# selftok-team/SelftokTokenizer

Hardware: NVIDIA H100
Metric: images/sec encode+50-step decode, 256x256/512-tok (higher is better)
Workload: dtype fp16 (IEEE-half operands on wgmma, fp32 accumulate; encoder/VQ/tables fp32)

## Files before the change

selftoktokenizer_b200/csrc/gemm_tc.cu:

```cuda
#include "common.cuh"
#include "hopper.cuh"
#include "kernels.h"

#include <stdlib.h>

namespace stk {

namespace {

using namespace hop;

constexpr int BM = 128, BN = 256, BK = 64, WK = 16;
constexpr int A_TILE_BYTES = BM * BK * 2;
constexpr int B_TILE_BYTES = BN * BK * 2;
constexpr int CONSUMERS = 2;
constexpr int NUM_THREADS = CONSUMERS * 128 + 128;
constexpr int PRODUCER_REGS = 40, CONSUMER_REGS = 232;
constexpr int ACC = BN / 2;
constexpr int kPrefetchKBlocks = 4;

template <int NSPLIT> struct Cfg {
  static constexpr int PLANES = NSPLIT == 3 ? 2 : 1;
  static constexpr int STAGE_BYTES = PLANES * (A_TILE_BYTES + B_TILE_BYTES);
  static constexpr int STAGES = NSPLIT == 3 ? 2 : 4;
  static constexpr int SMEM_BYTES = STAGES * STAGE_BYTES + 1024  + 256 ;
};

__device__ __forceinline__ void wgmma_tile(float (&d)[ACC], uint64_t da, uint64_t db, uint32_t acc, bool fp16) {
  if (fp16) wgmma_m64n256k16_ss_f16(d, da, db, acc);
  else wgmma_m64n256k16_ss_bf16(d, da, db, acc);
}

__device__ __forceinline__ float2 ldg2(const float* p) { return *reinterpret_cast<const float2*>(p); }

struct EpiRows {
  int orow[2], mrow[2];
  bool valid[2];
};

__device__ __forceinline__ EpiRows epilogue_rows(const Epilogue& e, int64_t row0, int64_t M) {
  const bool per_row_gate = e.mode == EPI_RESID && e.gate && (e.gate_period > 1 || e.tab_rows);
  const bool per_row_add = e.mode == EPI_STORE && e.addtab;
  EpiRows rw;
#pragma unroll
  for (int r = 0; r < 2; ++r) {
    const int64_t m = row0 + 8 * r;
    rw.valid[r] = m < M;
    const int mi = (int)m;
    rw.orow[r] = 0;
    if (e.row_map && rw.valid[r]) {
      rw.orow[r] = e.row_map[mi];
    } else if (e.plan && rw.valid[r]) {
      const int b = mi / e.rpb_in;
      const int n_img = e.rpb_out - (e.plan_ctx ? e.rpb_in : e.row_off);
      rw.orow[r] = b * e.rpb_out + plan_slot_row(mi % e.rpb_in, e.plan[2 * b], e.plan[2 * b + 1], n_img, e.plan_ctx != 0);
    } else if (rw.valid[r]) {
      rw.orow[r] = e.rpb_in > 0 ? (mi / e.rpb_in) * e.rpb_out + e.row_off + (mi % e.rpb_in) : mi;
    }
    if (e.tab_rows && rw.valid[r]) rw.mrow[r] = e.tab_rows[mi];
    else rw.mrow[r] = per_row_gate ? mi % e.gate_period : (per_row_add ? mi % e.add_period : 0);
  }
  return rw;
}

__device__ __forceinline__ void epilogue_prefetch(const Epilogue& e, const EpiRows& rw, int col0, int N) {
  if (e.mode != EPI_RESID) return;
  const int c0 = col0 & ~(BN - 1);
  const int q = (col0 >> 1) & 3;
#pragma unroll
  for (int r = 0; r < 2; ++r) {
#pragma unroll
    for (int h = 0; h < 2; ++h) {
      const int n = c0 + 32 * (2 * q + h);
      if (rw.valid[r] && n < N) prefetch_l2(e.resid + (int64_t)rw.orow[r] * e.ldo + n);
    }
  }
}

template <int MODE, bool GELU>
__device__ __forceinline__ void epilogue_tile(const Epilogue& e, const float (&acc)[ACC], const EpiRows& rw, int col0, int N) {
  constexpr int CH = MODE == EPI_RESID ? 4 : 8;
  const bool per_row_gate = MODE == EPI_RESID && e.gate && (e.gate_period > 1 || e.tab_rows);
  const bool per_row_add = MODE == EPI_STORE && e.addtab;
  const bool fp16 = e.fp16 != 0;
  const float2 zero = make_float2(0.f, 0.f), one = make_float2(1.f, 1.f);
#pragma unroll
  for (int c = 0; c < BN / 8; c += CH) {
    float2 bias[CH], res[2][CH], gt[2][CH], add[2][CH];
#pragma unroll
    for (int i = 0; i < CH; ++i) {
      const int n = col0 + 8 * (c + i);
      const bool in = n < N;
      bias[i] = e.bias && in ? ldg2(e.bias + n) : zero;
#pragma unroll
      for (int r = 0; r < 2; ++r) {
        const bool v = in && rw.valid[r];
        const int64_t o = (int64_t)rw.orow[r] * e.ldo + n;
        if (MODE == EPI_RESID) {
          res[r][i] = v ? ldg2(e.resid + o) : zero;
          gt[r][i] = v && e.gate ? ldg2(per_row_gate ? e.gate + (int64_t)rw.mrow[r] * e.gate_ld + n : e.gate + n) : one;
        }
        if (MODE == EPI_STORE) add[r][i] = v && per_row_add ? ldg2(e.addtab + (int64_t)rw.mrow[r] * e.add_ld + n) : zero;
      }
    }
#pragma unroll
    for (int i = 0; i < CH; ++i) {
      const int j = c + i;
      const int n = col0 + 8 * j;
      if (n >= N) continue;
#pragma unroll
      for (int r = 0; r < 2; ++r) {
        if (!rw.valid[r]) continue;
        float2 y = make_float2(acc[4 * j + 2 * r] + bias[i].x, acc[4 * j + 2 * r + 1] + bias[i].y);
        if (GELU) y = gelu_tanh_fast2(y);
        const int64_t o = (int64_t)rw.orow[r] * e.ldo + n;
        if (MODE == EPI_RESID) {
          y.x = fmaf(gt[r][i].x, y.x, res[r][i].x); y.y = fmaf(gt[r][i].y, y.y, res[r][i].y);
        }
        if (MODE == EPI_SPLIT) {
          const uint32_t hi = pack2_sat16(y.x, y.y, fp16);
          *reinterpret_cast<uint32_t*>(e.out_hi + o) = hi;
          if (e.out_lo) {
            const float lx = y.x - __bfloat162float(__float2bfloat16_rn(y.x)), ly = y.y - __bfloat162float(__float2bfloat16_rn(y.y));
            *reinterpret_cast<uint32_t*>(e.out_lo + o) = pack2_sat16(lx, ly, false);
          }
        } else {
          if (per_row_add) { y.x += add[r][i].x; y.y += add[r][i].y; }
          *reinterpret_cast<float2*>(e.out + o) = y;
        }
      }
    }
  }
}

__device__ __forceinline__ void epilogue_dispatch(const Epilogue& e, const float (&acc)[ACC], const EpiRows& rw, int col0, int N) {
  if (e.mode == EPI_RESID) epilogue_tile<EPI_RESID, false>(e, acc, rw, col0, N);
  else if (e.mode == EPI_SPLIT) {
    if (e.act == ACT_GELU) epilogue_tile<EPI_SPLIT, true>(e, acc, rw, col0, N);
    else epilogue_tile<EPI_SPLIT, false>(e, acc, rw, col0, N);
  } else {
    if (e.act == ACT_GELU) epilogue_tile<EPI_STORE, true>(e, acc, rw, col0, N);
    else epilogue_tile<EPI_STORE, false>(e, acc, rw, col0, N);
  }
}

struct TcMaps {
  CUtensorMap a_hi, a_lo, b_hi, b_lo;
};

struct GemmParams {
  int64_t M;
  int N, K;
  int fp16;
  Epilogue ep;
  int conv_C = 0, conv_H = 0, conv_W = 0, conv_stride = 1;
  int raster_gm = 4;
};

__device__ __forceinline__ void tile_coords(int t, int pm_tiles, int n_tiles, int GM, int& pm, int& n_blk) {
  const int per_group = GM * n_tiles;
  const int group = t / per_group;
  const int first = group * GM;
  const int gm = min(GM, pm_tiles - first);
  const int local = t - group * per_group;
  pm = first + local % gm;
  n_blk = local / gm;
}

template <int NSPLIT, int CL, bool FP16>
__global__ void __launch_bounds__(NUM_THREADS, 1)
gemm_tc_kernel(const __grid_constant__ TcMaps maps0, const __grid_constant__ TcMaps maps1, const GemmParams p0, const GemmParams p1) {
  static_assert(NSPLIT == 1 || !FP16, "the fp16 mode is single-pass");
  using C = Cfg<NSPLIT>;
  extern __shared__ uint8_t smem_raw[];
  const uint32_t smem_base = (smem_u32(smem_raw) + 1023u) & ~1023u;
  const uint32_t bar_base = smem_base + C::STAGES * C::STAGE_BYTES;
  auto full_bar = [&](int s) { return bar_base + 8u * s; };
  auto empty_bar = [&](int s) { return bar_base + 8u * (C::STAGES + s); };

  const int warp = threadIdx.x >> 5, lane = threadIdx.x & 31;
  const uint32_t rank = CL > 1 ? cluster_ctarank() : 0;
  const int pm_tiles0 = (int)((p0.M + CL * BM - 1) / (CL * BM)), n_tiles0 = (p0.N + BN - 1) / BN;
  const int pm_tiles1 = (int)((p1.M + CL * BM - 1) / (CL * BM)), n_tiles1 = (p1.N + BN - 1) / BN;
  const int tiles0 = pm_tiles0 * n_tiles0;
  const int num_tiles = tiles0 + pm_tiles1 * n_tiles1;
  const int cluster_id = blockIdx.x / CL, num_clusters = gridDim.x / CL;

  if (warp == CONSUMERS * 4 && lane == 0) {
    tma_prefetch_desc(&maps0.a_hi);
    tma_prefetch_desc(&maps0.b_hi);
    if (NSPLIT == 3) { tma_prefetch_desc(&maps0.a_lo); tma_prefetch_desc(&maps0.b_lo); }
    if (p1.M > 0) {
      tma_prefetch_desc(&maps1.a_hi);
      tma_prefetch_desc(&maps1.b_hi);
      if (NSPLIT == 3) { tma_prefetch_desc(&maps1.a_lo); tma_prefetch_desc(&maps1.b_lo); }
    }
    for (int s = 0; s < C::STAGES; ++s) { mbar_init(full_bar(s), 1); mbar_init(empty_bar(s), CONSUMERS * CL); }
    asm volatile("fence.mbarrier_init.release.cluster;" ::: "memory");
  }
  __syncthreads();
  if (CL > 1) cluster_sync_all();

  if (warp >= CONSUMERS * 4) {
    setmaxnreg_dec<PRODUCER_REGS>();
    if (warp == CONSUMERS * 4 && lane == 0) {
      int stage = 0; uint32_t phase = 0;
      const uint64_t w_policy = l2_policy_evict_last();
      for (int t = cluster_id; t < num_tiles; t += num_clusters) {
        const bool second = t >= tiles0;
        const TcMaps& mp = second ? maps1 : maps0;
        const GemmParams& pp = second ? p1 : p0;
        int pm, n_blk;
        if (second) tile_coords(t - tiles0, pm_tiles1, n_tiles1, p1.raster_gm, pm, n_blk);
        else tile_coords(t, pm_tiles0, n_tiles0, p0.raster_gm, pm, n_blk);
        const int nk = (pp.K + BK - 1) / BK;
        const int m_row = (pm * CL + (int)rank) * BM;
        const int n_row = n_blk * BN + (int)rank * (BN / CL);
        const int chunks = pp.conv_C > 0 ? pp.conv_C / BK : 1;
        int cx = 0, cy = 0, cb = 0;
        if (pp.conv_C > 0) {
          cx = m_row % pp.conv_W;
          cy = (m_row / pp.conv_W) % pp.conv_H;
          cb = m_row / (pp.conv_W * pp.conv_H);
        }
        for (int kb = 0; kb < nk; ++kb) {
          mbar_wait(empty_bar(stage), phase ^ 1);
          const uint32_t sa = smem_base + stage * C::STAGE_BYTES;
          const uint32_t sb = sa + C::PLANES * A_TILE_BYTES + (uint32_t)rank * (B_TILE_BYTES / CL);
          const uint32_t fb = full_bar(stage);
          mbar_expect_tx(fb, C::STAGE_BYTES);
          if (pp.conv_C > 0) {
            const int tap = kb / chunks, c0 = (kb - tap * chunks) * BK;
            const int dy = tap / 3, dx = tap - dy * 3;
            int x0 = cx + dx - 1, y0 = cy + dy - 1, n0 = cb;
            if (pp.conv_stride == 2) { x0 = cx + (dx >> 1); y0 = cy + (dy >> 1); n0 = cb * 4 + (dy & 1) * 2 + (dx & 1); }
            tma_load_4d(sa, &mp.a_hi, fb, c0, x0, y0, n0);
            if (NSPLIT == 3) tma_load_4d(sa + A_TILE_BYTES, &mp.a_lo, fb, c0, x0, y0, n0);
          } else {
            tma_load_2d(sa, &mp.a_hi, fb, kb * BK, m_row);
            if (NSPLIT == 3) tma_load_2d(sa + A_TILE_BYTES, &mp.a_lo, fb, kb * BK, m_row);
          }
          if (CL > 1) {
            tma_load_2d_mc(sb, &mp.b_hi, fb, kb * BK, n_row, (uint16_t)((1u << CL) - 1), w_policy);
            if (NSPLIT == 3) tma_load_2d_mc(sb + B_TILE_BYTES, &mp.b_lo, fb, kb * BK, n_row, (uint16_t)((1u << CL) - 1), w_policy);
          } else {
            tma_load_2d_hint(sb, &mp.b_hi, fb, kb * BK, n_row, w_policy);
            if (NSPLIT == 3) tma_load_2d_hint(sb + B_TILE_BYTES, &mp.b_lo, fb, kb * BK, n_row, w_policy);
          }
          if (++stage == C::STAGES) { stage = 0; phase ^= 1; }
        }
      }
    }
  } else {
    setmaxnreg_inc<CONSUMER_REGS>();
    const int wg = warp >> 2;
    const bool signaller = (threadIdx.x & 127) == 0;
    auto release = [&](int s) {
      if (!signaller) return;
      if (CL == 1) mbar_arrive(empty_bar(s));
      else for (int r = 0; r < CL; ++r) mbar_arrive_cluster(empty_bar(s), (uint32_t)r);
    };
    int stage = 0; uint32_t phase = 0;
    for (int t = cluster_id; t < num_tiles; t += num_clusters) {
      const bool second = t >= tiles0;
      int pm, n_blk;
      if (second) tile_coords(t - tiles0, pm_tiles1, n_tiles1, p1.raster_gm, pm, n_blk);
      else tile_coords(t, pm_tiles0, n_tiles0, p0.raster_gm, pm, n_blk);
      const int nk = ((second ? p1.K : p0.K) + BK - 1) / BK;
      const int wl = threadIdx.x & 127;
      const int64_t row0 = (int64_t)(pm * CL + (int)rank) * BM + wg * 64 + (wl >> 5) * 16 + ((wl & 31) >> 2);
      const int col0 = n_blk * BN + 2 * (wl & 3);
      const EpiRows rw = second ? epilogue_rows(p1.ep, row0, p1.M) : epilogue_rows(p0.ep, row0, p0.M);
      const int pf_kb = nk > kPrefetchKBlocks ? nk - kPrefetchKBlocks : 0;
      float acc[ACC];
#pragma unroll
      for (int i = 0; i < ACC; ++i) acc[i] = 0.f;
      int prev = -1;
      for (int kb = 0; kb < nk; ++kb) {
        mbar_wait(full_bar(stage), phase);
        const uint32_t sa_hi = smem_base + stage * C::STAGE_BYTES + wg * (64 * 128);
        const uint32_t sa_lo = sa_hi + A_TILE_BYTES;
        const uint32_t sb_hi = smem_base + stage * C::STAGE_BYTES + C::PLANES * A_TILE_BYTES;
        const uint32_t sb_lo = sb_hi + B_TILE_BYTES;
        wgmma_fence();
#pragma unroll
        for (int k = 0; k < BK / WK; ++k) {
          const uint32_t koff = k * WK * 2;
          const uint64_t da_hi = make_smem_desc(sa_hi + koff), db_hi = make_smem_desc(sb_hi + koff);
          wgmma_tile(acc, da_hi, db_hi, (kb > 0 || k > 0) ? 1u : 0u, FP16);
          if (NSPLIT == 3) {
            const uint64_t da_lo = make_smem_desc(sa_lo + koff), db_lo = make_smem_desc(sb_lo + koff);
            wgmma_tile(acc, da_hi, db_lo, 1u, false);
            wgmma_tile(acc, da_lo, db_hi, 1u, false);
          }
        }
        wgmma_commit();
        if (kb == pf_kb) {
          if (!second) epilogue_prefetch(p0.ep, rw, col0, p0.N);
          else epilogue_prefetch(p1.ep, rw, col0, p1.N);
        }
        wgmma_wait<1>();
        if (prev >= 0) release(prev);
        prev = stage;
        if (++stage == C::STAGES) { stage = 0; phase ^= 1; }
      }
      wgmma_wait<0>();
      fence_regs(acc);
      release(prev);
      if (!second) epilogue_dispatch(p0.ep, acc, rw, col0, p0.N);
      else epilogue_dispatch(p1.ep, acc, rw, col0, p1.N);
    }
  }
  if (CL > 1) cluster_sync_all();
}

typedef CUresult (*EncodeTiledFn)(CUtensorMap*, CUtensorMapDataType, cuuint32_t, void*, const cuuint64_t*, const cuuint64_t*,
                                  const cuuint32_t*, const cuuint32_t*, CUtensorMapInterleave, CUtensorMapSwizzle,
                                  CUtensorMapL2promotion, CUtensorMapFloatOOBfill);
EncodeTiledFn g_encode = nullptr;
constexpr int kMaxDev = 64;
int g_num_sms_dev[kMaxDev];
bool g_attr_dev[kMaxDev];
int g_raster_gm = 4;
int g_gemm_ctas = 2;

// ... 38 lines not shown
  cuuint64_t gdim[2] = {(cuuint64_t)cols, (cuuint64_t)rows};
  cuuint64_t gstride[1] = {(cuuint64_t)cols * 2};
  cuuint32_t box[2] = {box_cols, box_rows};
  cuuint32_t estr[2] = {1, 1};
  CUresult r = g_encode(map, fp16 ? CU_TENSOR_MAP_DATA_TYPE_FLOAT16 : CU_TENSOR_MAP_DATA_TYPE_BFLOAT16, 2, const_cast<void*>(ptr), gdim,
                        gstride, box, estr, CU_TENSOR_MAP_INTERLEAVE_NONE, CU_TENSOR_MAP_SWIZZLE_128B,
                        CU_TENSOR_MAP_L2_PROMOTION_L2_256B, CU_TENSOR_MAP_FLOAT_OOB_FILL_NONE);
  if (r != CUDA_SUCCESS) {
    set_error("cuTensorMapEncodeTiled failed with CUresult " + std::to_string((int)r));
    return -5;
  }
  return 0;
}

void gemm_tc_set_ctas(int n) { g_gemm_ctas = n == 1 ? 1 : 2; }

int gemm_tc_init() {
  int dev = 0;
  STK_CUDA(cudaGetDevice(&dev));
  STK_CHECK(dev >= 0 && dev < kMaxDev, -1, "gemm_tc: device ordinal out of range");
  if (g_encode && g_attr_dev[dev]) return 0;
  if (!g_encode) {
    void* fn = nullptr;
    cudaDriverEntryPointQueryResult qres;
    STK_CUDA(cudaGetDriverEntryPoint("cuTensorMapEncodeTiled", &fn, cudaEnableDefault, &qres));
    STK_CHECK(fn && qres == cudaDriverEntryPointSuccess, -5, "cuTensorMapEncodeTiled not available from the driver");
    const char* v = getenv("SELFTOK_GEMM_CTAS");
    if (v) g_gemm_ctas = atoi(v) == 1 ? 1 : 2;
    const char* gm = getenv("SELFTOK_GEMM_GM");
    if (gm && atoi(gm) >= 1 && atoi(gm) <= 1024) g_raster_gm = atoi(gm);
    g_encode = reinterpret_cast<EncodeTiledFn>(fn);
  }
  STK_CUDA(cudaDeviceGetAttribute(&g_num_sms_dev[dev], cudaDevAttrMultiProcessorCount, dev));
  STK_CUDA(cudaFuncSetAttribute(gemm_tc_kernel<1, 1, false>, cudaFuncAttributeMaxDynamicSharedMemorySize, Cfg<1>::SMEM_BYTES));
  STK_CUDA(cudaFuncSetAttribute(gemm_tc_kernel<1, 1, true>, cudaFuncAttributeMaxDynamicSharedMemorySize, Cfg<1>::SMEM_BYTES));
  STK_CUDA(cudaFuncSetAttribute(gemm_tc_kernel<3, 1, false>, cudaFuncAttributeMaxDynamicSharedMemorySize, Cfg<3>::SMEM_BYTES));
  STK_CUDA(cudaFuncSetAttribute(gemm_tc_kernel<1, 2, false>, cudaFuncAttributeMaxDynamicSharedMemorySize, Cfg<1>::SMEM_BYTES));
  STK_CUDA(cudaFuncSetAttribute(gemm_tc_kernel<1, 2, true>, cudaFuncAttributeMaxDynamicSharedMemorySize, Cfg<1>::SMEM_BYTES));
  STK_CUDA(cudaFuncSetAttribute(gemm_tc_kernel<3, 2, false>, cudaFuncAttributeMaxDynamicSharedMemorySize, Cfg<3>::SMEM_BYTES));
  g_attr_dev[dev] = true;
  return 0;
}

int check_gemm_tc_problem(const TcProblem& q, int nsplit, int fp16) {
  const Epilogue& ep = q.ep;
  STK_CHECK(q.A_hi && q.W_hi && q.M > 0 && q.N > 0 && q.K > 0, -1, "gemm_tc: bad arguments");
  STK_CHECK(nsplit == 1 || (nsplit == 3 && q.A_lo && q.W_lo), -1, "gemm_tc: nsplit must be 1, or 3 with lo planes");
  STK_CHECK(!fp16 || nsplit == 1, -1, "gemm_tc: the fp16 mode is single-pass");
  auto aligned16 = [](const void* p) { return reinterpret_cast<uintptr_t>(p) % 16 == 0; };
  STK_CHECK(aligned16(q.A_hi) && aligned16(q.A_lo) && aligned16(q.W_hi) && aligned16(q.W_lo), -1,
            "gemm_tc: operand planes must be 16-byte aligned (TMA)");
  STK_TRY(check_epilogue(ep, "gemm_tc"));
  STK_CHECK(ep.act == ACT_NONE || (ep.act == ACT_GELU && ep.mode != EPI_RESID), -2,
            "gemm_tc: epilogue activation must be none, or GELU-tanh with the store / split modes");
  STK_CHECK(ep.mode != EPI_STORE || ep.addtab == nullptr || ep.add_ld % 4 == 0, -2, "gemm_tc: addtab pitch must be a multiple of 4");
  STK_CHECK(q.K % 8 == 0, -2, "gemm_tc: K must be a multiple of 8 (16-byte TMA row pitch)");
  STK_CHECK(ep.ldo % 4 == 0 && q.N % 4 == 0, -2, "gemm_tc: N and the output pitch must be multiples of 4");
  STK_CHECK(ep.mode != EPI_RESID || ep.gate == nullptr || ep.gate_ld % 4 == 0, -2, "gemm_tc: gate pitch must be a multiple of 4");
  if (q.conv_C > 0) {
    STK_CHECK(q.conv_C % BK == 0 && q.K == 9 * q.conv_C, -2, "gemm_tc conv: channels must be a multiple of 64 and K = 9 C");
    STK_CHECK(q.conv_W > 0 && q.conv_H > 0 && (q.conv_W % BM == 0 || BM % q.conv_W == 0), -2, "gemm_tc conv: image width must divide or be a multiple of 128");
    const int64_t hw = (int64_t)q.conv_H * q.conv_W;
    STK_CHECK(q.M % hw == 0 && (hw % BM == 0 || BM % hw == 0) && (q.conv_W >= BM || hw < BM || q.conv_H % (BM / q.conv_W) == 0), -2,
              "gemm_tc conv: 128-pixel tiles must be part of a row, whole rows of one image, or whole images");
    STK_CHECK(q.conv_stride == 1 || (q.conv_stride == 2 && hw % BM == 0), -2, "gemm_tc conv: stride 2 needs >= 128 output pixels per image");
  }
  return 0;
}

static int make_maps(TcMaps* m, const TcProblem& q, int nsplit, int fp16, int b_box) {
  const bool conv = q.conv_C > 0;
  const int64_t imgs = conv ? q.M / ((int64_t)q.conv_H * q.conv_W) * (q.conv_stride == 2 ? 4 : 1) : 0;
  if (conv) STK_TRY(make_map_nhwc(&m->a_hi, q.A_hi, imgs, q.conv_H, q.conv_W, q.conv_C, fp16));
  else STK_TRY(make_map(&m->a_hi, q.A_hi, q.M, q.K, BM, fp16));
  STK_TRY(make_map(&m->b_hi, q.W_hi, q.N, q.K, b_box, fp16));
  if (nsplit == 3) {
    if (conv) STK_TRY(make_map_nhwc(&m->a_lo, q.A_lo, imgs, q.conv_H, q.conv_W, q.conv_C, fp16));
    else STK_TRY(make_map(&m->a_lo, q.A_lo, q.M, q.K, BM, fp16));
    STK_TRY(make_map(&m->b_lo, q.W_lo, q.N, q.K, b_box, fp16));
  } else {
    m->a_lo = m->a_hi; m->b_lo = m->b_hi;
  }
  return 0;
}

template <int NSPLIT, int CL, bool FP16>
static int launch_kernel(const TcMaps& m0, const TcMaps& m1, const GemmParams& p0, const GemmParams& p1, int clusters, cudaStream_t s) {
  cudaLaunchConfig_t cfg = {};
  cfg.gridDim = dim3(CL * clusters);
  cfg.blockDim = dim3(NUM_THREADS);
  cfg.dynamicSmemBytes = Cfg<NSPLIT>::SMEM_BYTES;
  cfg.stream = s;
  cudaLaunchAttribute attr[1];
  attr[0].id = cudaLaunchAttributeClusterDimension;
  attr[0].val.clusterDim.x = CL; attr[0].val.clusterDim.y = 1; attr[0].val.clusterDim.z = 1;
  cfg.attrs = attr;
  cfg.numAttrs = 1;
  STK_CUDA(cudaLaunchKernelEx(&cfg, gemm_tc_kernel<NSPLIT, CL, FP16>, m0, m1, p0, p1));
  count_launch();
  return 0;
}

template <int CL>
static int launch_cl(const TcMaps& m0, const TcMaps& m1, const GemmParams& p0, const GemmParams& p1, int clusters, int nsplit, int fp16,
                     cudaStream_t s) {
  if (nsplit == 3) return launch_kernel<3, CL, false>(m0, m1, p0, p1, clusters, s);
  if (fp16) return launch_kernel<1, CL, true>(m0, m1, p0, p1, clusters, s);
  return launch_kernel<1, CL, false>(m0, m1, p0, p1, clusters, s);
}

int launch_gemm_tc_grouped(const TcProblem* probs, int n, int nsplit, cudaStream_t s, int fp16) {
  STK_TRY(gemm_tc_init());
  STK_CHECK(probs && (n == 1 || n == 2), -1, "gemm_tc: one or two problems per launch");
  int dev = 0;
  STK_CUDA(cudaGetDevice(&dev));
  const int g_num_sms = g_num_sms_dev[dev];
  for (int i = 0; i < n; ++i) STK_TRY(check_gemm_tc_problem(probs[i], nsplit, fp16));
  const int CL = g_gemm_ctas == 2 && g_num_sms >= 2 ? 2 : 1;
  TcMaps m0, m1;
  STK_TRY(make_maps(&m0, probs[0], nsplit, fp16, BN / CL));
  auto mk_params = [&](const TcProblem& q) {
    GemmParams g{q.M, q.N, q.K, fp16, q.ep};
    g.conv_C = q.conv_C; g.conv_H = q.conv_H; g.conv_W = q.conv_W; g.conv_stride = q.conv_stride;
    g.raster_gm = g_raster_gm;
    return g;
  };
  GemmParams p0 = mk_params(probs[0]);
  GemmParams p1 = p0;
  p1.M = 0;
  m1 = m0;
  int tiles = (int)((probs[0].M + CL * BM - 1) / (CL * BM)) * ((probs[0].N + BN - 1) / BN);
  if (n == 2) {
    STK_TRY(make_maps(&m1, probs[1], nsplit, fp16, BN / CL));
    p1 = mk_params(probs[1]);
    tiles += (int)((probs[1].M + CL * BM - 1) / (CL * BM)) * ((probs[1].N + BN - 1) / BN);
  }
  const int clusters = tiles < g_num_sms / CL ? tiles : g_num_sms / CL;
  if (CL == 2) return launch_cl<2>(m0, m1, p0, p1, clusters, nsplit, fp16, s);
  return launch_cl<1>(m0, m1, p0, p1, clusters, nsplit, fp16, s);
}

int launch_gemm_tc(const __nv_bfloat16* A_hi, const __nv_bfloat16* A_lo, const __nv_bfloat16* W_hi,
                   const __nv_bfloat16* W_lo, int64_t M, int N, int K, int nsplit, const Epilogue& ep,
                   cudaStream_t s, int fp16) {
  TcProblem q{A_hi, A_lo, W_hi, W_lo, M, N, K, ep};
  return launch_gemm_tc_grouped(&q, 1, nsplit, s, fp16);
}

}
```

selftoktokenizer_b200/csrc/hopper.cuh:

```cuda
#pragma once
#include <cuda.h>
#include <stdint.h>

namespace stk {
namespace hop {

__device__ __forceinline__ uint32_t smem_u32(const void* p) { return (uint32_t)__cvta_generic_to_shared(p); }

__device__ __forceinline__ void mbar_init(uint32_t bar, uint32_t count) {
  asm volatile("mbarrier.init.shared::cta.b64 [%0], %1;" ::"r"(bar), "r"(count) : "memory");
}
__device__ __forceinline__ void mbar_expect_tx(uint32_t bar, uint32_t bytes) {
  asm volatile("mbarrier.arrive.expect_tx.shared::cta.b64 _, [%0], %1;" ::"r"(bar), "r"(bytes) : "memory");
}
__device__ __forceinline__ void mbar_arrive(uint32_t bar) {
  asm volatile("mbarrier.arrive.shared::cta.b64 _, [%0];" ::"r"(bar) : "memory");
}
__device__ __forceinline__ void mbar_arrive_cluster(uint32_t local_bar, uint32_t rank) {
  asm volatile(
      "{\n\t.reg .b32 ra;\n\t"
      "mapa.shared::cluster.u32 ra, %0, %1;\n\t"
      "mbarrier.arrive.shared::cluster.b64 _, [ra];\n\t}"
      ::"r"(local_bar), "r"(rank) : "memory");
}
// ... 81 lines not shown
  for (int i = 0; i < R; ++i) asm volatile("" : "+f"(d[i])::"memory");
}

#define STK_WGMMA_SS_N256(NAME, T)                                                                                   \
  __device__ __forceinline__ void NAME(float (&d)[128], uint64_t da, uint64_t db, uint32_t accumulate) { \
    asm volatile("{\n\t.reg .pred p;\n\tsetp.ne.b32 p, %130, 0;\n\t"                                             \
                 "wgmma.mma_async.sync.aligned.m64n256k16.f32." T "." T " "                                             \
                 "{%0, %1, %2, %3, %4, %5, %6, %7, %8, %9, %10, %11, %12, %13, %14, %15, %16, %17, %18, %19, %20, %21, %22, %23, %24, %25, %26, %27, %28, %29, %30, %31, %32, %33, %34, %35, %36, %37, %38, %39, %40, %41, %42, %43, %44, %45, %46, %47, %48, %49, %50, %51, %52, %53, %54, %55, %56, %57, %58, %59, %60, %61, %62, %63, %64, %65, %66, %67, %68, %69, %70, %71, %72, %73, %74, %75, %76, %77, %78, %79, %80, %81, %82, %83, %84, %85, %86, %87, %88, %89, %90, %91, %92, %93, %94, %95, %96, %97, %98, %99, %100, %101, %102, %103, %104, %105, %106, %107, %108, %109, %110, %111, %112, %113, %114, %115, %116, %117, %118, %119, %120, %121, %122, %123, %124, %125, %126, %127}, "  \
                 "%128, %129, p, 1, 1, 0, 0;\n\t}"                                                                  \
                 : "+f"(d[0]), "+f"(d[1]), "+f"(d[2]), "+f"(d[3]), "+f"(d[4]), "+f"(d[5]), "+f"(d[6]), "+f"(d[7]), "+f"(d[8]), "+f"(d[9]), "+f"(d[10]), "+f"(d[11]), "+f"(d[12]), "+f"(d[13]), "+f"(d[14]), "+f"(d[15]), "+f"(d[16]), "+f"(d[17]), "+f"(d[18]), "+f"(d[19]), "+f"(d[20]), "+f"(d[21]), "+f"(d[22]), "+f"(d[23]), "+f"(d[24]), "+f"(d[25]), "+f"(d[26]), "+f"(d[27]), "+f"(d[28]), "+f"(d[29]), "+f"(d[30]), "+f"(d[31]), "+f"(d[32]), "+f"(d[33]), "+f"(d[34]), "+f"(d[35]), "+f"(d[36]), "+f"(d[37]), "+f"(d[38]), "+f"(d[39]), "+f"(d[40]), "+f"(d[41]), "+f"(d[42]), "+f"(d[43]), "+f"(d[44]), "+f"(d[45]), "+f"(d[46]), "+f"(d[47]), "+f"(d[48]), "+f"(d[49]), "+f"(d[50]), "+f"(d[51]), "+f"(d[52]), "+f"(d[53]), "+f"(d[54]), "+f"(d[55]), "+f"(d[56]), "+f"(d[57]), "+f"(d[58]), "+f"(d[59]), "+f"(d[60]), "+f"(d[61]), "+f"(d[62]), "+f"(d[63]), "+f"(d[64]), "+f"(d[65]), "+f"(d[66]), "+f"(d[67]), "+f"(d[68]), "+f"(d[69]), "+f"(d[70]), "+f"(d[71]), "+f"(d[72]), "+f"(d[73]), "+f"(d[74]), "+f"(d[75]), "+f"(d[76]), "+f"(d[77]), "+f"(d[78]), "+f"(d[79]), "+f"(d[80]), "+f"(d[81]), "+f"(d[82]), "+f"(d[83]), "+f"(d[84]), "+f"(d[85]), "+f"(d[86]), "+f"(d[87]), "+f"(d[88]), "+f"(d[89]), "+f"(d[90]), "+f"(d[91]), "+f"(d[92]), "+f"(d[93]), "+f"(d[94]), "+f"(d[95]), "+f"(d[96]), "+f"(d[97]), "+f"(d[98]), "+f"(d[99]), "+f"(d[100]), "+f"(d[101]), "+f"(d[102]), "+f"(d[103]), "+f"(d[104]), "+f"(d[105]), "+f"(d[106]), "+f"(d[107]), "+f"(d[108]), "+f"(d[109]), "+f"(d[110]), "+f"(d[111]), "+f"(d[112]), "+f"(d[113]), "+f"(d[114]), "+f"(d[115]), "+f"(d[116]), "+f"(d[117]), "+f"(d[118]), "+f"(d[119]), "+f"(d[120]), "+f"(d[121]), "+f"(d[122]), "+f"(d[123]), "+f"(d[124]), "+f"(d[125]), "+f"(d[126]), "+f"(d[127]) \
                 : "l"(da), "l"(db), "r"(accumulate));                                                                         \
  }
STK_WGMMA_SS_N256(wgmma_m64n256k16_ss_bf16, "bf16")
STK_WGMMA_SS_N256(wgmma_m64n256k16_ss_f16, "f16")

#define STK_WGMMA_SS_N64(NAME, T)                                                                                   \
  __device__ __forceinline__ void NAME(float (&d)[32], uint64_t da, uint64_t db, uint32_t accumulate) { \
    asm volatile("{\n\t.reg .pred p;\n\tsetp.ne.b32 p, %34, 0;\n\t"                                             \
                 "wgmma.mma_async.sync.aligned.m64n64k16.f32." T "." T " "                                             \
                 "{%0, %1, %2, %3, %4, %5, %6, %7, %8, %9, %10, %11, %12, %13, %14, %15, %16, %17, %18, %19, %20, %21, %22, %23, %24, %25, %26, %27, %28, %29, %30, %31}, "  \
                 "%32, %33, p, 1, 1, 0, 0;\n\t}"                                                                  \
                 : "+f"(d[0]), "+f"(d[1]), "+f"(d[2]), "+f"(d[3]), "+f"(d[4]), "+f"(d[5]), "+f"(d[6]), "+f"(d[7]), "+f"(d[8]), "+f"(d[9]), "+f"(d[10]), "+f"(d[11]), "+f"(d[12]), "+f"(d[13]), "+f"(d[14]), "+f"(d[15]), "+f"(d[16]), "+f"(d[17]), "+f"(d[18]), "+f"(d[19]), "+f"(d[20]), "+f"(d[21]), "+f"(d[22]), "+f"(d[23]), "+f"(d[24]), "+f"(d[25]), "+f"(d[26]), "+f"(d[27]), "+f"(d[28]), "+f"(d[29]), "+f"(d[30]), "+f"(d[31]) \
                 : "l"(da), "l"(db), "r"(accumulate));                                                                         \
  }
STK_WGMMA_SS_N64(wgmma_m64n64k16_ss_bf16, "bf16")
STK_WGMMA_SS_N64(wgmma_m64n64k16_ss_f16, "f16")

#define STK_WGMMA_RS_N64(NAME, T)                                                                                   \
  __device__ __forceinline__ void NAME(float (&d)[32], const uint32_t (&a)[4], uint64_t db, uint32_t accumulate) { \
    asm volatile("{\n\t.reg .pred p;\n\tsetp.ne.b32 p, %37, 0;\n\t"                                             \
// ... 12 lines not shown
```

Measured before the change: 9.979.

## Add ping-pong consumer schedule with 128x128 tiles to the wgmma GEMM

Adds a ping-pong mode in which the two consumer warpgroups take alternate output tiles of 128x128. Each warpgroup computes a full tile with two m64n128 wgmmas, and an mbarrier token passes MMA issue between them so one group's epilogue can overlap the other's main loop. The mode is picked per launch when K is at most 3072 and the epilogue is not residual, and it is always used for bf16x3. It uses more pipeline stages with smaller weight tiles. It also adds a host-side check that the A planes do not overlap the output. The tradeoff is that halving the tile width gives less weight reuse per loaded A tile, and the epilogue now handles four row groups.

Measured after the change: 10.05, median of 6. No clear change (+0.7%).

```diff
diff --git a/selftoktokenizer_b200/csrc/gemm_tc.cu b/selftoktokenizer_b200/csrc/gemm_tc.cu
--- a/selftoktokenizer_b200/csrc/gemm_tc.cu
+++ b/selftoktokenizer_b200/csrc/gemm_tc.cu
@@ -10,41 +10,44 @@
 
 using namespace hop;
 
-constexpr int BM = 128, BN = 256, BK = 64, WK = 16;
+constexpr int BM = 128, BK = 64, WK = 16;
 constexpr int A_TILE_BYTES = BM * BK * 2;
-constexpr int B_TILE_BYTES = BN * BK * 2;
 constexpr int CONSUMERS = 2;
 constexpr int NUM_THREADS = CONSUMERS * 128 + 128;
 constexpr int PRODUCER_REGS = 40, CONSUMER_REGS = 232;
-constexpr int ACC = BN / 2;
+constexpr int ACC = 128;
 constexpr int kPrefetchKBlocks = 4;
-
-template <int NSPLIT> struct Cfg {
+constexpr int kPingPongMaxK = 3072;
+
+template <int NSPLIT, bool PP> struct Cfg {
+  static_assert(PP || NSPLIT == 1, "bf16x3 always runs the ping-pong schedule");
   static constexpr int PLANES = NSPLIT == 3 ? 2 : 1;
-  static constexpr int STAGE_BYTES = PLANES * (A_TILE_BYTES + B_TILE_BYTES);
-  static constexpr int STAGES = NSPLIT == 3 ? 2 : 4;
+  static constexpr int TILE_N = PP ? 128 : 256;
+  static constexpr int W_TILE_BYTES = TILE_N * BK * 2;
+  static constexpr int STAGE_BYTES = PLANES * (A_TILE_BYTES + W_TILE_BYTES);
+  static constexpr int STAGES = PP ? (NSPLIT == 3 ? 3 : 6) : 4;
   static constexpr int SMEM_BYTES = STAGES * STAGE_BYTES + 1024  + 256 ;
+  static constexpr int ROWS = PP ? 4 : 2;
 };
 
-__device__ __forceinline__ void wgmma_tile(float (&d)[ACC], uint64_t da, uint64_t db, uint32_t acc, bool fp16) {
-  if (fp16) wgmma_m64n256k16_ss_f16(d, da, db, acc);
-  else wgmma_m64n256k16_ss_bf16(d, da, db, acc);
-}
-
 __device__ __forceinline__ float2 ldg2(const float* p) { return *reinterpret_cast<const float2*>(p); }
 
-struct EpiRows {
-  int orow[2], mrow[2];
-  bool valid[2];
+__device__ __forceinline__ int epi_row_offset(int r) { return 8 * (r & 1) + 64 * (r >> 1); }
+__device__ __forceinline__ int epi_acc_index(int r, int j) { return 64 * (r >> 1) + 4 * j + 2 * (r & 1); }
+
+template <int ROWS> struct EpiRows {
+  int orow[ROWS], mrow[ROWS];
+  bool valid[ROWS];
 };
 
-__device__ __forceinline__ EpiRows epilogue_rows(const Epilogue& e, int64_t row0, int64_t M) {
+template <int ROWS>
+__device__ __forceinline__ EpiRows<ROWS> epilogue_rows(const Epilogue& e, int64_t row0, int64_t M) {
   const bool per_row_gate = e.mode == EPI_RESID && e.gate && (e.gate_period > 1 || e.tab_rows);
   const bool per_row_add = e.mode == EPI_STORE && e.addtab;
-  EpiRows rw;
-#pragma unroll
-  for (int r = 0; r < 2; ++r) {
-    const int64_t m = row0 + 8 * r;
+  EpiRows<ROWS> rw;
+#pragma unroll
+  for (int r = 0; r < ROWS; ++r) {
+    const int64_t m = row0 + epi_row_offset(r);
     rw.valid[r] = m < M;
     const int mi = (int)m;
     rw.orow[r] = 0;
@@ -63,37 +66,40 @@
   return rw;
 }
 
-__device__ __forceinline__ void epilogue_prefetch(const Epilogue& e, const EpiRows& rw, int col0, int N) {
+template <int ROWS>
+__device__ __forceinline__ void epilogue_prefetch(const Epilogue& e, const EpiRows<ROWS>& rw, int col0, int N) {
+  constexpr int PAIRS = 64 / ROWS, LINES = PAIRS / 16;
   if (e.mode != EPI_RESID) return;
-  const int c0 = col0 & ~(BN - 1);
+  const int c0 = col0 & ~(8 * PAIRS - 1);
   const int q = (col0 >> 1) & 3;
 #pragma unroll
-  for (int r = 0; r < 2; ++r) {
-#pragma unroll
-    for (int h = 0; h < 2; ++h) {
-      const int n = c0 + 32 * (2 * q + h);
+  for (int r = 0; r < ROWS; ++r) {
+#pragma unroll
+    for (int h = 0; h < LINES; ++h) {
+      const int n = c0 + 32 * (LINES * q + h);
       if (rw.valid[r] && n < N) prefetch_l2(e.resid + (int64_t)rw.orow[r] * e.ldo + n);
     }
   }
 }
 
-template <int MODE, bool GELU>
-__device__ __forceinline__ void epilogue_tile(const Epilogue& e, const float (&acc)[ACC], const EpiRows& rw, int col0, int N) {
-  constexpr int CH = MODE == EPI_RESID ? 4 : 8;
+template <int ROWS, int MODE, bool GELU>
+__device__ __forceinline__ void epilogue_tile(const Epilogue& e, const float (&acc)[ACC], const EpiRows<ROWS>& rw, int col0, int N) {
+  constexpr int PAIRS = 64 / ROWS;
+  constexpr int CH = (MODE == EPI_RESID ? 8 : 16) / ROWS;
   const bool per_row_gate = MODE == EPI_RESID && e.gate && (e.gate_period > 1 || e.tab_rows);
   const bool per_row_add = MODE == EPI_STORE && e.addtab;
   const bool fp16 = e.fp16 != 0;
   const float2 zero = make_float2(0.f, 0.f), one = make_float2(1.f, 1.f);
 #pragma unroll
-  for (int c = 0; c < BN / 8; c += CH) {
-    float2 bias[CH], res[2][CH], gt[2][CH], add[2][CH];
+  for (int c = 0; c < PAIRS; c += CH) {
+    float2 bias[CH], res[ROWS][CH], gt[ROWS][CH], add[ROWS][CH];
 #pragma unroll
     for (int i = 0; i < CH; ++i) {
       const int n = col0 + 8 * (c + i);
       const bool in = n < N;
       bias[i] = e.bias && in ? ldg2(e.bias + n) : zero;
 #pragma unroll
-      for (int r = 0; r < 2; ++r) {
+      for (int r = 0; r < ROWS; ++r) {
         const bool v = in && rw.valid[r];
         const int64_t o = (int64_t)rw.orow[r] * e.ldo + n;
         if (MODE == EPI_RESID) {
@@ -109,9 +115,10 @@
       const int n = col0 + 8 * j;
       if (n >= N) continue;
 #pragma unroll
-      for (int r = 0; r < 2; ++r) {
+      for (int r = 0; r < ROWS; ++r) {
         if (!rw.valid[r]) continue;
-        float2 y = make_float2(acc[4 * j + 2 * r] + bias[i].x, acc[4 * j + 2 * r + 1] + bias[i].y);
+        const int a = epi_acc_index(r, j);
+        float2 y = make_float2(acc[a] + bias[i].x, acc[a + 1] + bias[i].y);
         if (GELU) y = gelu_tanh_fast2(y);
         const int64_t o = (int64_t)rw.orow[r] * e.ldo + n;
         if (MODE == EPI_RESID) {
@@ -133,14 +140,43 @@
   }
 }
 
-__device__ __forceinline__ void epilogue_dispatch(const Epilogue& e, const float (&acc)[ACC], const EpiRows& rw, int col0, int N) {
-  if (e.mode == EPI_RESID) epilogue_tile<EPI_RESID, false>(e, acc, rw, col0, N);
+template <int ROWS>
+__device__ __forceinline__ void epilogue_dispatch(const Epilogue& e, const float (&acc)[ACC], const EpiRows<ROWS>& rw, int col0, int N) {
+  if (e.mode == EPI_RESID) epilogue_tile<ROWS, EPI_RESID, false>(e, acc, rw, col0, N);
   else if (e.mode == EPI_SPLIT) {
-    if (e.act == ACT_GELU) epilogue_tile<EPI_SPLIT, true>(e, acc, rw, col0, N);
-    else epilogue_tile<EPI_SPLIT, false>(e, acc, rw, col0, N);
+    if (e.act == ACT_GELU) epilogue_tile<ROWS, EPI_SPLIT, true>(e, acc, rw, col0, N);
+    else epilogue_tile<ROWS, EPI_SPLIT, false>(e, acc, rw, col0, N);
   } else {
-    if (e.act == ACT_GELU) epilogue_tile<EPI_STORE, true>(e, acc, rw, col0, N);
-    else epilogue_tile<EPI_STORE, false>(e, acc, rw, col0, N);
+    if (e.act == ACT_GELU) epilogue_tile<ROWS, EPI_STORE, true>(e, acc, rw, col0, N);
+    else epilogue_tile<ROWS, EPI_STORE, false>(e, acc, rw, col0, N);
+  }
+}
+
+template <bool PP, int NSPLIT, bool FP16>
+__device__ __forceinline__ void mma_k16(float (&acc)[ACC], uint32_t sa_hi, uint32_t sa_lo, uint32_t sb_hi, uint32_t sb_lo,
+                                        uint32_t accumulate) {
+  const uint64_t db_hi = make_smem_desc(sb_hi);
+#pragma unroll
+  for (int h = 0; h < (PP ? 2 : 1); ++h) {
+    const uint64_t da_hi = make_smem_desc(sa_hi + h * (64 * 128));
+    float (&d)[64] = *reinterpret_cast<float (*)[64]>(&acc[64 * h]);
+    if (PP) {
+      if (FP16) wgmma_m64n128k16_ss_f16(d, da_hi, db_hi, accumulate);
+      else wgmma_m64n128k16_ss_bf16(d, da_hi, db_hi, accumulate);
+    } else {
+      if (FP16) wgmma_m64n256k16_ss_f16(acc, da_hi, db_hi, accumulate);
+      else wgmma_m64n256k16_ss_bf16(acc, da_hi, db_hi, accumulate);
+    }
+    if (NSPLIT == 3) {
+      const uint64_t da_lo = make_smem_desc(sa_lo + h * (64 * 128)), db_lo = make_smem_desc(sb_lo);
+      if (PP) {
+        wgmma_m64n128k16_ss_bf16(d, da_hi, db_lo, 1u);
+        wgmma_m64n128k16_ss_bf16(d, da_lo, db_hi, 1u);
+      } else {
+        wgmma_m64n256k16_ss_bf16(acc, da_hi, db_lo, 1u);
+        wgmma_m64n256k16_ss_bf16(acc, da_lo, db_hi, 1u);
+      }
+    }
   }
 }
 
@@ -167,23 +203,26 @@
   n_blk = local / gm;
 }
 
-template <int NSPLIT, int CL, bool FP16>
+template <int NSPLIT, int CL, bool FP16, bool PP>
 __global__ void __launch_bounds__(NUM_THREADS, 1)
 gemm_tc_kernel(const __grid_constant__ TcMaps maps0, const __grid_constant__ TcMaps maps1, const GemmParams p0, const GemmParams p1) {
   static_assert(NSPLIT == 1 || !FP16, "the fp16 mode is single-pass");
-  using C = Cfg<NSPLIT>;
+  using C = Cfg<NSPLIT, PP>;
+  constexpr int TILE_N = C::TILE_N;
   extern __shared__ uint8_t smem_raw[];
   const uint32_t smem_base = (smem_u32(smem_raw) + 1023u) & ~1023u;
   const uint32_t bar_base = smem_base + C::STAGES * C::STAGE_BYTES;
   auto full_bar = [&](int s) { return bar_base + 8u * s; };
   auto empty_bar = [&](int s) { return bar_base + 8u * (C::STAGES + s); };
+  auto mma_bar = [&](int w) { return bar_base + 8u * (2 * C::STAGES + w); };
 
   const int warp = threadIdx.x >> 5, lane = threadIdx.x & 31;
   const uint32_t rank = CL > 1 ? cluster_ctarank() : 0;
-  const int pm_tiles0 = (int)((p0.M + CL * BM - 1) / (CL * BM)), n_tiles0 = (p0.N + BN - 1) / BN;
-  const int pm_tiles1 = (int)((p1.M + CL * BM - 1) / (CL * BM)), n_tiles1 = (p1.N + BN - 1) / BN;
+  const int pm_tiles0 = (int)((p0.M + CL * BM - 1) / (CL * BM)), n_tiles0 = (p0.N + TILE_N - 1) / TILE_N;
+  const int pm_tiles1 = (int)((p1.M + CL * BM - 1) / (CL * BM)), n_tiles1 = (p1.N + TILE_N - 1) / TILE_N;
   const int tiles0 = pm_tiles0 * n_tiles0;
   const int num_tiles = tiles0 + pm_tiles1 * n_tiles1;
+  const int nk0 = (p0.K + BK - 1) / BK, nk1 = (p1.K + BK - 1) / BK;
   const int cluster_id = blockIdx.x / CL, num_clusters = gridDim.x / CL;
 
   if (warp == CONSUMERS * 4 && lane == 0) {
@@ -195,7 +234,8 @@
       tma_prefetch_desc(&maps1.b_hi);
       if (NSPLIT == 3) { tma_prefetch_desc(&maps1.a_lo); tma_prefetch_desc(&maps1.b_lo); }
     }
-    for (int s = 0; s < C::STAGES; ++s) { mbar_init(full_bar(s), 1); mbar_init(empty_bar(s), CONSUMERS * CL); }
+    for (int s = 0; s < C::STAGES; ++s) { mbar_init(full_bar(s), 1); mbar_init(empty_bar(s), (PP ? 1 : CONSUMERS) * CL); }
+    for (int w = 0; w < CONSUMERS; ++w) mbar_init(mma_bar(w), 128);
     asm volatile("fence.mbarrier_init.release.cluster;" ::: "memory");
   }
   __syncthreads();
@@ -213,9 +253,9 @@
         int pm, n_blk;
         if (second) tile_coords(t - tiles0, pm_tiles1, n_tiles1, p1.raster_gm, pm, n_blk);
         else tile_coords(t, pm_tiles0, n_tiles0, p0.raster_gm, pm, n_blk);
-        const int nk = (pp.K + BK - 1) / BK;
+        const int nk = second ? nk1 : nk0;
         const int m_row = (pm * CL + (int)rank) * BM;
-        const int n_row = n_blk * BN + (int)rank * (BN / CL);
+        const int n_row = n_blk * TILE_N + (int)rank * (TILE_N / CL);
         const int chunks = pp.conv_C > 0 ? pp.conv_C / BK : 1;
         int cx = 0, cy = 0, cb = 0;
         if (pp.conv_C > 0) {
@@ -226,7 +266,7 @@
         for (int kb = 0; kb < nk; ++kb) {
           mbar_wait(empty_bar(stage), phase ^ 1);
           const uint32_t sa = smem_base + stage * C::STAGE_BYTES;
-          const uint32_t sb = sa + C::PLANES * A_TILE_BYTES + (uint32_t)rank * (B_TILE_BYTES / CL);
+          const uint32_t sb = sa + C::PLANES * A_TILE_BYTES + (uint32_t)rank * (C::W_TILE_BYTES / CL);
           const uint32_t fb = full_bar(stage);
           mbar_expect_tx(fb, C::STAGE_BYTES);
           if (pp.conv_C > 0) {
@@ -242,10 +282,10 @@
           }
           if (CL > 1) {
             tma_load_2d_mc(sb, &mp.b_hi, fb, kb * BK, n_row, (uint16_t)((1u << CL) - 1), w_policy);
-            if (NSPLIT == 3) tma_load_2d_mc(sb + B_TILE_BYTES, &mp.b_lo, fb, kb * BK, n_row, (uint16_t)((1u << CL) - 1), w_policy);
+            if (NSPLIT == 3) tma_load_2d_mc(sb + C::W_TILE_BYTES, &mp.b_lo, fb, kb * BK, n_row, (uint16_t)((1u << CL) - 1), w_policy);
           } else {
             tma_load_2d_hint(sb, &mp.b_hi, fb, kb * BK, n_row, w_policy);
-            if (NSPLIT == 3) tma_load_2d_hint(sb + B_TILE_BYTES, &mp.b_lo, fb, kb * BK, n_row, w_policy);
+            if (NSPLIT == 3) tma_load_2d_hint(sb + C::W_TILE_BYTES, &mp.b_lo, fb, kb * BK, n_row, w_policy);
           }
           if (++stage == C::STAGES) { stage = 0; phase ^= 1; }
         }
@@ -254,61 +294,68 @@
   } else {
     setmaxnreg_inc<CONSUMER_REGS>();
     const int wg = warp >> 2;
-    const bool signaller = (threadIdx.x & 127) == 0;
+    const int wl = threadIdx.x & 127;
+    const bool signaller = wl == 0;
     auto release = [&](int s) {
       if (!signaller) return;
       if (CL == 1) mbar_arrive(empty_bar(s));
       else for (int r = 0; r < CL; ++r) mbar_arrive_cluster(empty_bar(s), (uint32_t)r);
     };
-    int stage = 0; uint32_t phase = 0;
-    for (int t = cluster_id; t < num_tiles; t += num_clusters) {
+    if (PP && wg == 1) mbar_arrive(mma_bar(0));
+    int stage = 0; uint32_t phase = 0, turn = 0;
+    int slot = 0;
+    for (int t = cluster_id; t < num_tiles; t += num_clusters, slot ^= 1) {
       const bool second = t >= tiles0;
+      const int nk = second ? nk1 : nk0;
+      if (PP && slot != wg) {
+        stage += nk;
+        const int wraps = stage / C::STAGES;
+        stage -= wraps * C::STAGES;
+        phase ^= (uint32_t)(wraps & 1);
+        continue;
+      }
       int pm, n_blk;
       if (second) tile_coords(t - tiles0, pm_tiles1, n_tiles1, p1.raster_gm, pm, n_blk);
       else tile_coords(t, pm_tiles0, n_tiles0, p0.raster_gm, pm, n_blk);
-      const int nk = ((second ? p1.K : p0.K) + BK - 1) / BK;
-      const int wl = threadIdx.x & 127;
-      const int64_t row0 = (int64_t)(pm * CL + (int)rank) * BM + wg * 64 + (wl >> 5) * 16 + ((wl & 31) >> 2);
-      const int col0 = n_blk * BN + 2 * (wl & 3);
-      const EpiRows rw = second ? epilogue_rows(p1.ep, row0, p1.M) : epilogue_rows(p0.ep, row0, p0.M);
+      const int wg_row = PP ? 0 : 64 * wg;
+      const int64_t row0 = (int64_t)(pm * CL + (int)rank) * BM + wg_row + (wl >> 5) * 16 + ((wl & 31) >> 2);
+      const int col0 = n_blk * TILE_N + 2 * (wl & 3);
+      const EpiRows<C::ROWS> rw = second ? epilogue_rows<C::ROWS>(p1.ep, row0, p1.M) : epilogue_rows<C::ROWS>(p0.ep, row0, p0.M);
       const int pf_kb = nk > kPrefetchKBlocks ? nk - kPrefetchKBlocks : 0;
       float acc[ACC];
 #pragma unroll
       for (int i = 0; i < ACC; ++i) acc[i] = 0.f;
+      if (PP) mbar_wait(mma_bar(wg), turn);
       int prev = -1;
       for (int kb = 0; kb < nk; ++kb) {
         mbar_wait(full_bar(stage), phase);
-        const uint32_t sa_hi = smem_base + stage * C::STAGE_BYTES + wg * (64 * 128);
+        const uint32_t sa_hi = smem_base + stage * C::STAGE_BYTES + wg_row * 128;
         const uint32_t sa_lo = sa_hi + A_TILE_BYTES;
         const uint32_t sb_hi = smem_base + stage * C::STAGE_BYTES + C::PLANES * A_TILE_BYTES;
-        const uint32_t sb_lo = sb_hi + B_TILE_BYTES;
+        const uint32_t sb_lo = sb_hi + C::W_TILE_BYTES;
         wgmma_fence();
 #pragma unroll
         for (int k = 0; k < BK / WK; ++k) {
           const uint32_t koff = k * WK * 2;
-          const uint64_t da_hi = make_smem_desc(sa_hi + koff), db_hi = make_smem_desc(sb_hi + koff);
-          wgmma_tile(acc, da_hi, db_hi, (kb > 0 || k > 0) ? 1u : 0u, FP16);
-          if (NSPLIT == 3) {
-            const uint64_t da_lo = make_smem_desc(sa_lo + koff), db_lo = make_smem_desc(sb_lo + koff);
-            wgmma_tile(acc, da_hi, db_lo, 1u, false);
-            wgmma_tile(acc, da_lo, db_hi, 1u, false);
-          }
+          mma_k16<PP, NSPLIT, FP16>(acc, sa_hi + koff, sa_lo + koff, sb_hi + koff, sb_lo + koff, (kb > 0 || k > 0) ? 1u : 0u);
         }
         wgmma_commit();
         if (kb == pf_kb) {
-          if (!second) epilogue_prefetch(p0.ep, rw, col0, p0.N);
-          else epilogue_prefetch(p1.ep, rw, col0, p1.N);
+          if (!second) epilogue_prefetch<C::ROWS>(p0.ep, rw, col0, p0.N);
+          else epilogue_prefetch<C::ROWS>(p1.ep, rw, col0, p1.N);
         }
         wgmma_wait<1>();
         if (prev >= 0) release(prev);
         prev = stage;
         if (++stage == C::STAGES) { stage = 0; phase ^= 1; }
       }
+      if (PP) mbar_arrive(mma_bar(wg ^ 1));
+      turn ^= 1;
       wgmma_wait<0>();
       fence_regs(acc);
       release(prev);
-      if (!second) epilogue_dispatch(p0.ep, acc, rw, col0, p0.N);
-      else epilogue_dispatch(p1.ep, acc, rw, col0, p1.N);
+      if (!second) epilogue_dispatch<C::ROWS>(p0.ep, acc, rw, col0, p0.N);
+      else epilogue_dispatch<C::ROWS>(p1.ep, acc, rw, col0, p1.N);
     }
   }
   if (CL > 1) cluster_sync_all();
@@ -377,6 +424,12 @@
 }
 
 void gemm_tc_set_ctas(int n) { g_gemm_ctas = n == 1 ? 1 : 2; }
+
+template <int NSPLIT, int CL, bool FP16, bool PP>
+static int set_smem_attr() {
+  STK_CUDA(cudaFuncSetAttribute(gemm_tc_kernel<NSPLIT, CL, FP16, PP>, cudaFuncAttributeMaxDynamicSharedMemorySize, Cfg<NSPLIT, PP>::SMEM_BYTES));
+  return 0;
+}
 
 int gemm_tc_init() {
   int dev = 0;
@@ -395,12 +448,16 @@
     g_encode = reinterpret_cast<EncodeTiledFn>(fn);
   }
   STK_CUDA(cudaDeviceGetAttribute(&g_num_sms_dev[dev], cudaDevAttrMultiProcessorCount, dev));
-  STK_CUDA(cudaFuncSetAttribute(gemm_tc_kernel<1, 1, false>, cudaFuncAttributeMaxDynamicSharedMemorySize, Cfg<1>::SMEM_BYTES));
-  STK_CUDA(cudaFuncSetAttribute(gemm_tc_kernel<1, 1, true>, cudaFuncAttributeMaxDynamicSharedMemorySize, Cfg<1>::SMEM_BYTES));
-  STK_CUDA(cudaFuncSetAttribute(gemm_tc_kernel<3, 1, false>, cudaFuncAttributeMaxDynamicSharedMemorySize, Cfg<3>::SMEM_BYTES));
-  STK_CUDA(cudaFuncSetAttribute(gemm_tc_kernel<1, 2, false>, cudaFuncAttributeMaxDynamicSharedMemorySize, Cfg<1>::SMEM_BYTES));
-  STK_CUDA(cudaFuncSetAttribute(gemm_tc_kernel<1, 2, true>, cudaFuncAttributeMaxDynamicSharedMemorySize, Cfg<1>::SMEM_BYTES));
-  STK_CUDA(cudaFuncSetAttribute(gemm_tc_kernel<3, 2, false>, cudaFuncAttributeMaxDynamicSharedMemorySize, Cfg<3>::SMEM_BYTES));
+  STK_TRY((set_smem_attr<1, 1, false, true>()));
+  STK_TRY((set_smem_attr<1, 1, false, false>()));
+  STK_TRY((set_smem_attr<1, 1, true, true>()));
+  STK_TRY((set_smem_attr<1, 1, true, false>()));
+  STK_TRY((set_smem_attr<3, 1, false, true>()));
+  STK_TRY((set_smem_attr<1, 2, false, true>()));
+  STK_TRY((set_smem_attr<1, 2, false, false>()));
+  STK_TRY((set_smem_attr<1, 2, true, true>()));
+  STK_TRY((set_smem_attr<1, 2, true, false>()));
+  STK_TRY((set_smem_attr<3, 2, false, true>()));
   g_attr_dev[dev] = true;
   return 0;
 }
@@ -428,6 +485,19 @@
               "gemm_tc conv: 128-pixel tiles must be part of a row, whole rows of one image, or whole images");
     STK_CHECK(q.conv_stride == 1 || (q.conv_stride == 2 && hw % BM == 0), -2, "gemm_tc conv: stride 2 needs >= 128 output pixels per image");
   }
+  const int64_t a_elems = q.conv_C > 0 ? q.M * q.conv_C * (q.conv_stride == 2 ? 4 : 1) : q.M * (int64_t)q.K;
+  const int64_t out_rows = ep.rpb_in > 0 ? std::max(q.M, (q.M + ep.rpb_in - 1) / ep.rpb_in * ep.rpb_out) : q.M;
+  const int64_t out_elems = (out_rows - 1) * ep.ldo + q.N;
+  auto overlap = [](const void* a, int64_t a_bytes, const void* b, int64_t b_bytes) {
+    const uintptr_t a0 = reinterpret_cast<uintptr_t>(a), b0 = reinterpret_cast<uintptr_t>(b);
+    return a && b && a0 < b0 + (uintptr_t)b_bytes && b0 < a0 + (uintptr_t)a_bytes;
+  };
+  const void* outs[3] = {ep.mode == EPI_SPLIT ? nullptr : ep.out, ep.mode == EPI_SPLIT ? ep.out_hi : nullptr,
+                         ep.mode == EPI_SPLIT ? ep.out_lo : nullptr};
+  const int64_t out_bytes[3] = {4 * out_elems, 2 * out_elems, 2 * out_elems};
+  for (int i = 0; i < 3; ++i)
+    STK_CHECK(!overlap(q.A_hi, 2 * a_elems, outs[i], out_bytes[i]) && !(nsplit == 3 && overlap(q.A_lo, 2 * a_elems, outs[i], out_bytes[i])),
+              -1, "gemm_tc: the A planes must not overlap the output");
   return 0;
 }
 
@@ -447,29 +517,33 @@
   return 0;
 }
 
-template <int NSPLIT, int CL, bool FP16>
+template <int NSPLIT, int CL, bool FP16, bool PP>
 static int launch_kernel(const TcMaps& m0, const TcMaps& m1, const GemmParams& p0, const GemmParams& p1, int clusters, cudaStream_t s) {
   cudaLaunchConfig_t cfg = {};
   cfg.gridDim = dim3(CL * clusters);
   cfg.blockDim = dim3(NUM_THREADS);
-  cfg.dynamicSmemBytes = Cfg<NSPLIT>::SMEM_BYTES;
+  cfg.dynamicSmemBytes = Cfg<NSPLIT, PP>::SMEM_BYTES;
   cfg.stream = s;
   cudaLaunchAttribute attr[1];
   attr[0].id = cudaLaunchAttributeClusterDimension;
   attr[0].val.clusterDim.x = CL; attr[0].val.clusterDim.y = 1; attr[0].val.clusterDim.z = 1;
   cfg.attrs = attr;
   cfg.numAttrs = 1;
-  STK_CUDA(cudaLaunchKernelEx(&cfg, gemm_tc_kernel<NSPLIT, CL, FP16>, m0, m1, p0, p1));
+  STK_CUDA(cudaLaunchKernelEx(&cfg, gemm_tc_kernel<NSPLIT, CL, FP16, PP>, m0, m1, p0, p1));
   count_launch();
   return 0;
 }
 
-template <int CL>
+template <int CL, bool PP>
 static int launch_cl(const TcMaps& m0, const TcMaps& m1, const GemmParams& p0, const GemmParams& p1, int clusters, int nsplit, int fp16,
                      cudaStream_t s) {
-  if (nsplit == 3) return launch_kernel<3, CL, false>(m0, m1, p0, p1, clusters, s);
-  if (fp16) return launch_kernel<1, CL, true>(m0, m1, p0, p1, clusters, s);
-  return launch_kernel<1, CL, false>(m0, m1, p0, p1, clusters, s);
+  if (nsplit == 3) return launch_kernel<3, CL, false, true>(m0, m1, p0, p1, clusters, s);
+  if (fp16) return launch_kernel<1, CL, true, PP>(m0, m1, p0, p1, clusters, s);
+  return launch_kernel<1, CL, false, PP>(m0, m1, p0, p1, clusters, s);
+}
+
+static bool pingpong_pays(const TcProblem& q, int nsplit) {
+  return nsplit == 3 || (q.K <= kPingPongMaxK && q.ep.mode != EPI_RESID);
 }
 
 int launch_gemm_tc_grouped(const TcProblem* probs, int n, int nsplit, cudaStream_t s, int fp16) {
@@ -480,8 +554,10 @@
   const int g_num_sms = g_num_sms_dev[dev];
   for (int i = 0; i < n; ++i) STK_TRY(check_gemm_tc_problem(probs[i], nsplit, fp16));
   const int CL = g_gemm_ctas == 2 && g_num_sms >= 2 ? 2 : 1;
+  const bool pp = pingpong_pays(probs[0], nsplit) && (n == 1 || pingpong_pays(probs[1], nsplit));
+  const int tile_n = pp ? Cfg<1, true>::TILE_N : Cfg<1, false>::TILE_N;
   TcMaps m0, m1;
-  STK_TRY(make_maps(&m0, probs[0], nsplit, fp16, BN / CL));
+  STK_TRY(make_maps(&m0, probs[0], nsplit, fp16, tile_n / CL));
   auto mk_params = [&](const TcProblem& q) {
     GemmParams g{q.M, q.N, q.K, fp16, q.ep};
     g.conv_C = q.conv_C; g.conv_H = q.conv_H; g.conv_W = q.conv_W; g.conv_stride = q.conv_stride;
@@ -492,15 +568,15 @@
   GemmParams p1 = p0;
   p1.M = 0;
   m1 = m0;
-  int tiles = (int)((probs[0].M + CL * BM - 1) / (CL * BM)) * ((probs[0].N + BN - 1) / BN);
+  int tiles = (int)((probs[0].M + CL * BM - 1) / (CL * BM)) * ((probs[0].N + tile_n - 1) / tile_n);
   if (n == 2) {
-    STK_TRY(make_maps(&m1, probs[1], nsplit, fp16, BN / CL));
+    STK_TRY(make_maps(&m1, probs[1], nsplit, fp16, tile_n / CL));
     p1 = mk_params(probs[1]);
-    tiles += (int)((probs[1].M + CL * BM - 1) / (CL * BM)) * ((probs[1].N + BN - 1) / BN);
+    tiles += (int)((probs[1].M + CL * BM - 1) / (CL * BM)) * ((probs[1].N + tile_n - 1) / tile_n);
   }
   const int clusters = tiles < g_num_sms / CL ? tiles : g_num_sms / CL;
-  if (CL == 2) return launch_cl<2>(m0, m1, p0, p1, clusters, nsplit, fp16, s);
-  return launch_cl<1>(m0, m1, p0, p1, clusters, nsplit, fp16, s);
+  if (CL == 2) return pp ? launch_cl<2, true>(m0, m1, p0, p1, clusters, nsplit, fp16, s) : launch_cl<2, false>(m0, m1, p0, p1, clusters, nsplit, fp16, s);
+  return pp ? launch_cl<1, true>(m0, m1, p0, p1, clusters, nsplit, fp16, s) : launch_cl<1, false>(m0, m1, p0, p1, clusters, nsplit, fp16, s);
 }
 
 int launch_gemm_tc(const __nv_bfloat16* A_hi, const __nv_bfloat16* A_lo, const __nv_bfloat16* W_hi,
diff --git a/selftoktokenizer_b200/csrc/hopper.cuh b/selftoktokenizer_b200/csrc/hopper.cuh
--- a/selftoktokenizer_b200/csrc/hopper.cuh
+++ b/selftoktokenizer_b200/csrc/hopper.cuh
@@ -119,6 +119,18 @@
 STK_WGMMA_SS_N256(wgmma_m64n256k16_ss_bf16, "bf16")
 STK_WGMMA_SS_N256(wgmma_m64n256k16_ss_f16, "f16")
 
+#define STK_WGMMA_SS_N128(NAME, T)                                                                                   \
+  __device__ __forceinline__ void NAME(float (&d)[64], uint64_t da, uint64_t db, uint32_t accumulate) { \
+    asm volatile("{\n\t.reg .pred p;\n\tsetp.ne.b32 p, %66, 0;\n\t"                                             \
+                 "wgmma.mma_async.sync.aligned.m64n128k16.f32." T "." T " "                                             \
+                 "{%0, %1, %2, %3, %4, %5, %6, %7, %8, %9, %10, %11, %12, %13, %14, %15, %16, %17, %18, %19, %20, %21, %22, %23, %24, %25, %26, %27, %28, %29, %30, %31, %32, %33, %34, %35, %36, %37, %38, %39, %40, %41, %42, %43, %44, %45, %46, %47, %48, %49, %50, %51, %52, %53, %54, %55, %56, %57, %58, %59, %60, %61, %62, %63}, "  \
+                 "%64, %65, p, 1, 1, 0, 0;\n\t}"                                                                  \
+                 : "+f"(d[0]), "+f"(d[1]), "+f"(d[2]), "+f"(d[3]), "+f"(d[4]), "+f"(d[5]), "+f"(d[6]), "+f"(d[7]), "+f"(d[8]), "+f"(d[9]), "+f"(d[10]), "+f"(d[11]), "+f"(d[12]), "+f"(d[13]), "+f"(d[14]), "+f"(d[15]), "+f"(d[16]), "+f"(d[17]), "+f"(d[18]), "+f"(d[19]), "+f"(d[20]), "+f"(d[21]), "+f"(d[22]), "+f"(d[23]), "+f"(d[24]), "+f"(d[25]), "+f"(d[26]), "+f"(d[27]), "+f"(d[28]), "+f"(d[29]), "+f"(d[30]), "+f"(d[31]), "+f"(d[32]), "+f"(d[33]), "+f"(d[34]), "+f"(d[35]), "+f"(d[36]), "+f"(d[37]), "+f"(d[38]), "+f"(d[39]), "+f"(d[40]), "+f"(d[41]), "+f"(d[42]), "+f"(d[43]), "+f"(d[44]), "+f"(d[45]), "+f"(d[46]), "+f"(d[47]), "+f"(d[48]), "+f"(d[49]), "+f"(d[50]), "+f"(d[51]), "+f"(d[52]), "+f"(d[53]), "+f"(d[54]), "+f"(d[55]), "+f"(d[56]), "+f"(d[57]), "+f"(d[58]), "+f"(d[59]), "+f"(d[60]), "+f"(d[61]), "+f"(d[62]), "+f"(d[63]) \
+                 : "l"(da), "l"(db), "r"(accumulate));                                                                         \
+  }
+STK_WGMMA_SS_N128(wgmma_m64n128k16_ss_bf16, "bf16")
+STK_WGMMA_SS_N128(wgmma_m64n128k16_ss_f16, "f16")
+
 #define STK_WGMMA_SS_N64(NAME, T)                                                                                   \
   __device__ __forceinline__ void NAME(float (&d)[32], uint64_t da, uint64_t db, uint32_t accumulate) { \
     asm volatile("{\n\t.reg .pred p;\n\tsetp.ne.b32 p, %34, 0;\n\t"                                             \
```
